# HpWang-whu/YOHO

Hardware: AMD Instinct MI355X
Metric: keypoints/sec (5000 kp x60 rot desc+YOHO-O) (higher is better)
Workload: dtype fp16x2 split (2^-22-accurate products, fp32 accumulate); 1 GPU

## Files before the change

### yoho_amd/csrc/gemmf.h

```cpp
#pragma once
#include <hip/hip_runtime.h>
#include <type_traits>
#include "common.h"

namespace yoho {

typedef float floatx16 __attribute__((ext_vector_type(16)));
typedef float floatx4 __attribute__((ext_vector_type(4)));
typedef unsigned uintx4 __attribute__((ext_vector_type(4)));
typedef _Float16 halfx8 __attribute__((ext_vector_type(8)));
typedef const __attribute__((address_space(1))) void* gptr_t;
typedef __attribute__((address_space(3))) void* lptr_t;

constexpr int FG_STAGE = 32768;
constexpr int FG_LDS = 4 * FG_STAGE;

static const int FG_ORD_D[NIR_ORD] = {5, 4, 3, 3, 1};
static const int FG_ORD_R[NIR_ORD] = {4, 3, 1, 2, 0};
static const int FG_IR_BASE[5] = {0, 1, 10, 19, 35};
static const int FG_IR_D[5] = {1, 3, 3, 4, 5};

struct FGemmArgs {
    const char* A;
    const char* B;
// ... 43 lines not shown
    int start = 0;
    for (int u = 0; u < NIR_ORD; ++u) {
        const int ru = (xcd + a.rot[u]) & 7;
        const int cnt = a.NT[u] > ru ? ((a.NT[u] - 1 - ru) / 8 + 1) * a.MT[u] : 0;
        if (slot < start + cnt) { t = u; local = slot - start; r = ru; return true; }
        start += cnt;
    }
    return false;
}

inline int fgemm_grid(const FGemmArgs& a, int per_tile) {
    int tot = 0;
    for (int x = 0; x < 8; ++x) {
        int n = 0;
        for (int t = 0; t < NIR_ORD; ++t) {
            const int r = (x + a.rot[t]) & 7;
            if (a.NT[t] > r) n += ((a.NT[t] - 1 - r) / 8 + 1) * a.MT[t] * per_tile;
        }
        tot = n > tot ? n : tot;
    }
    return 8 * tot;
}

enum { F2_NOSTORE = 0x100, F2_MIX = 0x200, F2_ST_SC1 = 0x400, F2_ST_NT = 0x800, F2_SPARSE4 = 0x1000, F2_SPARSE16 = 0x2000, F2_K32 = 0x4000 };

__device__ __forceinline__ size_t slab_off(int tile32, int q, int cout8, int o, int half, int kp32) {
    return (((((size_t)tile32 * G + q) * cout8 + (o >> 3)) * 2 + half) * TILE + kp32) * 4;
}

template <int MI, int NJ>
__device__ __forceinline__ void residual_start(floatx16 (&acc)[MI][NJ], int row0, int kp0, int jidx, int d, int qbase, const float* res, float descale,
                                               int cout, int nT32, int lane) {
    const float inv = 1.f / descale;
    const int half = lane >> 5, kp32 = lane & 31, cout8 = cout >> 3;
#pragma unroll
    for (int bi = 0; bi < NJ; ++bi) {
        const int tile32 = (kp0 >> 5) + bi;
#pragma unroll
        for (int ai = 0; ai < MI; ++ai) {
            const int rowb = row0 + ai * 32;
            const int iidx = rowb / cout, o0 = rowb - iidx * cout;
            const bool ok = tile32 < nT32 && iidx < d;
            const int q = qbase + iidx * d + jidx;
#pragma unroll
            for (int q4 = 0; q4 < 4; ++q4) {
                const size_t off = slab_off(tile32, q, cout8, o0 + q4 * 8 + half * 4, half, kp32);
                const floatx4 v = *reinterpret_cast<const floatx4*>(res + (ok ? off : 0)) * (ok ? inv : 0.f);
                acc[ai][bi][4 * q4 + 0] = v.x; acc[ai][bi][4 * q4 + 1] = v.y;
                acc[ai][bi][4 * q4 + 2] = v.z; acc[ai][bi][4 * q4 + 3] = v.w;
            }
        }
    }
}

template <int MI, int NJ>
__device__ __forceinline__ void coef_epilogue(const floatx16 (&acc)[MI][NJ], int row0, int kp0, int jidx, int d, int qbase, float* out, const float* bias,
                                              float descale, int cout, int nT32, int* rflag, int lane, int flags) {
    const int half = lane >> 5, kp32 = lane & 31, cout8 = cout >> 3;
    unsigned top = 0u;
#ifdef YOHO_EXPERIMENTS
    if ((flags & F2_SPARSE4) && (blockIdx.x >> 3) % 4 != 0) flags |= F2_NOSTORE;
    if ((flags & F2_SPARSE16) && (blockIdx.x >> 3) % 16 != 0) flags |= F2_NOSTORE;
    const __amdgpu_buffer_rsrc_t orsrc = __builtin_amdgcn_make_buffer_rsrc(out, 0, 0x7FFFFFFF, 0x00020000);
#endif
#pragma unroll
    for (int bi = 0; bi < NJ; ++bi) {
        const int tile32 = (kp0 >> 5) + bi;
        if (tile32 >= nT32) continue;
#pragma unroll
        for (int ai = 0; ai < MI; ++ai) {
            const int rowb = row0 + ai * 32;
            const int iidx = rowb / cout, o0 = rowb - iidx * cout;
            if (iidx >= d) continue;
            const int q = qbase + iidx * d + jidx;
#pragma unroll
            for (int q4 = 0; q4 < 4; ++q4) {
                const int o = o0 + q4 * 8 + half * 4;
                floatx4 val;
                val.x = acc[ai][bi][4 * q4 + 0]; val.y = acc[ai][bi][4 * q4 + 1];
                val.z = acc[ai][bi][4 * q4 + 2]; val.w = acc[ai][bi][4 * q4 + 3];
                val *= descale;
                if (d == 1) val += *reinterpret_cast<const floatx4*>(bias + o) * 7.745966692414834f;
                const size_t off = slab_off(tile32, q, cout8, o, half, kp32);
#ifdef YOHO_EXPERIMENTS
                if (flags & F2_ST_SC1) __builtin_amdgcn_raw_buffer_store_b128(__builtin_bit_cast(uintx4, val), orsrc, (int)(off * 4), 0, 16);
                else if (flags & F2_ST_NT) __builtin_amdgcn_raw_buffer_store_b128(__builtin_bit_cast(uintx4, val), orsrc, (int)(off * 4), 0, 2);
                else if (!(flags & F2_NOSTORE))
#endif
                *reinterpret_cast<floatx4*>(out + off) = val;
                top = max(max(top, __float_as_uint(val.x) & 0x7FFFFFFFu), __float_as_uint(val.y) & 0x7FFFFFFFu);
                top = max(max(top, __float_as_uint(val.z) & 0x7FFFFFFFu), __float_as_uint(val.w) & 0x7FFFFFFFu);
            }
        }
    }
    note_range_bits(rflag, top, FP16_MAX / HF_ASCALE);
}

__device__ __forceinline__ floatx4 mfma_h16(uintx4 a, uintx4 b, floatx4 c) {
    union { uintx4 u; halfx8 h; } ca, cb;
    ca.u = a; cb.u = b;
    return __builtin_amdgcn_mfma_f32_16x16x32_f16(ca.h, cb.h, c, 0, 0, 0);
}

inline bool fgemm_layer_k32(const FGemmArgs& a) { return a.cin >= 256 && a.cin % 64 == 0 && a.cout >= 256; }

template <int NJ, typename Extra>
__device__ __forceinline__ void row_products32(floatx4 (&accrow)[NJ], const uintx4& al, const uintx4& ah, const uintx4 (&bh)[NJ], const uintx4 (&bl)[NJ],
                                               Extra&& extra) {
    sfor<0, 3 * NJ>([&](auto mc) {
        constexpr int m = decltype(mc)::value, j = m % NJ, p = m / NJ;
        accrow[j] = mfma_h16(p == 0 ? al : ah, p == 1 ? bl[j] : bh[j], accrow[j]);
        __builtin_amdgcn_sched_barrier(0);
        extra(mc);
        __builtin_amdgcn_sched_barrier(0);
    });
}

template <int LOB, int MI, int NJ>
// ... 21 lines not shown
#pragma unroll
    for (int i = 0; i < MI; ++i)
#pragma unroll
        for (int j = 0; j < NJ; ++j) acc[i][j] = floatx4{0.f, 0.f, 0.f, 0.f};
}

template <bool TO_SLAB>
__device__ __forceinline__ void swap_rows16(floatx4& x, floatx4& y) {
    typedef unsigned uintx2 __attribute__((ext_vector_type(2)));
#pragma unroll
    for (int e = 0; e < 4; ++e) {
        uintx2 r = {__float_as_uint(x[e]), __float_as_uint(y[e])};
        if constexpr (TO_SLAB) {
            r = __builtin_amdgcn_permlane16_swap(r.x, r.y, false, false);
            r = __builtin_amdgcn_permlane32_swap(r.x, r.y, false, false);
        } else {
            r = __builtin_amdgcn_permlane32_swap(r.x, r.y, false, false);
            r = __builtin_amdgcn_permlane16_swap(r.x, r.y, false, false);
        }
        x[e] = __uint_as_float(r.x); y[e] = __uint_as_float(r.y);
    }
}

template <int MI, int NJ>
__device__ __forceinline__ void residual_start(floatx4 (&acc)[MI][NJ], int row0, int kp0, int jidx, int d, int qbase, const float* res, float descale,
                                               int cout, int nT32, int lane) {
    static_assert(NJ % 2 == 0, "pairs of 16-column tiles");
    const float inv = 1.f / descale;
    const int half = lane >> 5, kp32 = lane & 31, cout8 = cout >> 3;
#pragma unroll
    for (int bi = 0; bi < NJ; bi += 2) {
        const int tile32 = (kp0 >> 5) + (bi >> 1);
#pragma unroll
        for (int ai = 0; ai < MI; ++ai) {
            const int rowb = row0 + ai * 16;
            const int iidx = rowb / cout, o0 = rowb - iidx * cout;
            const bool ok = tile32 < nT32 && iidx < d;
            const int q = qbase + iidx * d + jidx;
            const size_t off0 = slab_off(tile32, q, cout8, o0 + half * 4, half, kp32), off1 = slab_off(tile32, q, cout8, o0 + 8 + half * 4, half, kp32);
            acc[ai][bi] = *reinterpret_cast<const floatx4*>(res + (ok ? off0 : 0)) * (ok ? inv : 0.f);
            acc[ai][bi + 1] = *reinterpret_cast<const floatx4*>(res + (ok ? off1 : 0)) * (ok ? inv : 0.f);
            swap_rows16<false>(acc[ai][bi], acc[ai][bi + 1]);
        }
    }
}

template <int MI, int NJ>
__device__ __forceinline__ void coef_epilogue(const floatx4 (&acc)[MI][NJ], int row0, int kp0, int jidx, int d, int qbase, float* out, const float* bias,
                                              float descale, int cout, int nT32, int* rflag, int lane, int flags) {
    static_assert(NJ % 2 == 0, "pairs of 16-column tiles");
    const int half = lane >> 5, kp32 = lane & 31, cout8 = cout >> 3;
    unsigned top = 0u;
#pragma unroll
    for (int bi = 0; bi < NJ; bi += 2) {
        const int tile32 = (kp0 >> 5) + (bi >> 1);
        if (tile32 >= nT32) continue;
#pragma unroll
        for (int ai = 0; ai < MI; ++ai) {
            const int rowb = row0 + ai * 16;
            const int iidx = rowb / cout, o0 = rowb - iidx * cout;
            if (iidx >= d) continue;
            const int q = qbase + iidx * d + jidx;
            floatx4 v[2] = {acc[ai][bi], acc[ai][bi + 1]};
            swap_rows16<true>(v[0], v[1]);
#pragma unroll
            for (int h8 = 0; h8 < 2; ++h8) {
                const int o = o0 + h8 * 8 + half * 4;
                floatx4 val = v[h8] * descale;
                if (d == 1) val += *reinterpret_cast<const floatx4*>(bias + o) * 7.745966692414834f;
#ifdef YOHO_EXPERIMENTS
                if (!(flags & F2_NOSTORE))
#endif
                *reinterpret_cast<floatx4*>(out + slab_off(tile32, q, cout8, o, half, kp32)) = val;
                top = max(max(top, __float_as_uint(val.x) & 0x7FFFFFFFu), __float_as_uint(val.y) & 0x7FFFFFFFu);
                top = max(max(top, __float_as_uint(val.z) & 0x7FFFFFFFu), __float_as_uint(val.w) & 0x7FFFFFFFu);
            }
        }
    }
    note_range_bits(rflag, top, FP16_MAX / HF_ASCALE);
}

void fgemm_fill_args(FGemmArgs& a, const Layer& L, const char* Bplanes, int kppad, int nT32, const float* res, float* out, int* rflag);
int launch_fgemm2(const FGemmArgs& a, int flags, hipStream_t s);
int launch_fgemm3(const FGemmArgs& a, int flags, hipStream_t s);
int fgemm2_init();

}
```

### yoho_amd/csrc/gemmf.hip

```cpp
#include <hip/hip_runtime.h>
#include <hip/hip_fp16.h>
#include <type_traits>
#include <vector>
#include <cmath>
#include <cstring>
#include <cstdlib>

#include "common.h"
#include "gemmf.h"

namespace yoho {

struct Frags {
    uintx4 ah[4], al[4], bh[4], bl[4];
};

template <int SUB, int R>
__device__ __forceinline__ void read_frag(const char* pa, const char* pb, Frags& f) {
    constexpr int t = R & 3;
    if constexpr (R < 4) f.al[t] = *reinterpret_cast<const uintx4*>(pa + (2 + SUB) * 8192 + t * 512);
    else if constexpr (R < 8) f.bh[t] = *reinterpret_cast<const uintx4*>(pb + (0 + SUB) * 8192 + t * 512);
    else if constexpr (R < 12) f.ah[t] = *reinterpret_cast<const uintx4*>(pa + (0 + SUB) * 8192 + t * 512);
    else f.bl[t] = *reinterpret_cast<const uintx4*>(pb + (2 + SUB) * 8192 + t * 512);
}
// ... 54 lines not shown
    const int d = a.dim[t];
    const int MT = a.MT[t], KS = d * a.cin / 32;
    const int cg = local / MT, mtile = local - cg * MT;
    const int ntile = r + 8 * cg;
    const char* Ag = a.A + a.a_off[t] + (size_t)mtile * KS * FG_STAGE;
    const char* Bg = a.B + a.b_off[t] + (size_t)ntile * KS * FG_STAGE;
    const int wm = w >> 1, wn = w & 1;
    const int lane16 = lane * 16;
    const int row0 = mtile * 256 + wm * 128;
    const int col0 = ntile * 256 + wn * 128;

    floatx16 acc[4][4];
    zero_acc(acc);

    const int lane_a = (lane >> 5) * 4096 + (wm * 128 + (lane & 31)) * 16;
    const int lane_b = FG_STAGE + (lane >> 5) * 4096 + (wn * 128 + (lane & 31)) * 16;

    stage_tile(Ag, smem, w, lane);
    stage_tile(Bg, smem + FG_STAGE, w, lane);
    if (KS > 1) {
        stage_tile(Ag + FG_STAGE, smem + 2 * FG_STAGE, w, lane);
        stage_tile(Bg + FG_STAGE, smem + 3 * FG_STAGE, w, lane);
    }
    if ((flags & EPI_RES) && row0 < d * a.cout) residual_start(acc, row0, col0 % a.kppad, col0 / a.kppad, d, a.qbase[t], a.res, a.descale, a.cout, a.nT32, lane);
    asm volatile("s_waitcnt vmcnt(0)" ::: "memory");
    __syncthreads();

    if (row0 >= d * a.cout) {
        for (int s = 0; s < KS; ++s) {
            asm volatile("s_waitcnt vmcnt(0)" ::: "memory");
            __syncthreads();
            const int s2 = s + 2 < KS ? s + 2 : KS - 1;
            char* cur = smem + (s & 1) * (2 * FG_STAGE);
            stage_tile(Ag + (size_t)s2 * FG_STAGE, cur, w, lane);
            stage_tile(Bg + (size_t)s2 * FG_STAGE, cur + FG_STAGE, w, lane);
        }
        asm volatile("s_waitcnt vmcnt(0)" ::: "memory");
        return;
    }
    Frags P, Q;
    read_frags<0>(smem + lane_a, smem + lane_b, P);
    for (int s = 0; s < KS; ++s) {
        char* cur = smem + (s & 1) * (2 * FG_STAGE);
        char* nxt = smem + ((s + 1) & 1) * (2 * FG_STAGE);
        substep<1, false>(P, acc, cur + lane_a, cur + lane_b, Q, nullptr, nullptr, nullptr, w, lane16);
        asm volatile("s_waitcnt vmcnt(0) lgkmcnt(0)" ::: "memory");
        __syncthreads();
        __builtin_amdgcn_sched_barrier(0);
        const int s2 = s + 2 < KS ? s + 2 : KS - 1;
        substep<0, true>(Q, acc, nxt + lane_a, nxt + lane_b, P, uniform_ptr(Ag + (size_t)s2 * FG_STAGE), uniform_ptr(Bg + (size_t)s2 * FG_STAGE),
                              cur, w, lane16);
    }
    asm volatile("s_waitcnt vmcnt(0)" ::: "memory");

    coef_epilogue(acc, row0, col0 % a.kppad, col0 / a.kppad, d, a.qbase[t], a.out, a.bias, a.descale, a.cout, a.nT32, a.rflag, lane, flags);
}

__global__ __launch_bounds__(256, 1) void fgemmk_kernel(FGemmArgs a, int flags) {
    extern __shared__ __attribute__((aligned(16))) char smem[];
    const int tid = threadIdx.x, lane = tid & 63;
    const int w = __builtin_amdgcn_readfirstlane(tid >> 6);
    int t = 0, local = 0, r = 0;
    if (!fg3_map(a, blockIdx.x & 7, blockIdx.x >> 3, t, local, r)) return;
    const int d = a.dim[t];
    const int MT = a.MT[t], KS = d * a.cin / 32;
    const int cg = local / MT, mtile = local - cg * MT;
    const int ntile = r + 8 * cg;
    const char* Ag = a.A + a.a_off[t] + (size_t)mtile * KS * FG_STAGE;
    const char* Bg = a.B + a.b_off[t] + (size_t)ntile * KS * FG_STAGE;
    const int wm = w >> 1, wn = w & 1;
    const int row0 = mtile * 256 + wm * 128, col0 = ntile * 256 + wn * 128;
    const bool rows_live = row0 < d * a.cout;
    const int lane_a = (lane >> 4) * 4096 + (wm * 128 + (lane & 15)) * 16;
    const int lane_b = FG_STAGE + (lane >> 4) * 4096 + (wn * 128 + (lane & 15)) * 16;

    floatx4 acc[8][8];
    zero_acc(acc);
    stage_tile(Ag, smem, w, lane);
    stage_tile(Bg, smem + FG_STAGE, w, lane);
    if (KS > 1) {
        stage_tile(Ag + FG_STAGE, smem + 2 * FG_STAGE, w, lane);
        stage_tile(Bg + FG_STAGE, smem + 3 * FG_STAGE, w, lane);
    }
    if ((flags & EPI_RES) && rows_live) residual_start(acc, row0, col0 % a.kppad, col0 / a.kppad, d, a.qbase[t], a.res, a.descale, a.cout, a.nT32, lane);
    asm volatile("s_waitcnt vmcnt(0)" ::: "memory");
    __syncthreads();
    for (int s = 0; s < KS; ++s) {
        char* cur = smem + (s & 1) * (2 * FG_STAGE);
        if (rows_live) stage32_plain<FG_STAGE / 2>(acc, cur + lane_a, cur + lane_b);
        asm volatile("s_waitcnt vmcnt(0) lgkmcnt(0)" ::: "memory");
        __syncthreads();
        __builtin_amdgcn_sched_barrier(0);
        if (s + 2 < KS) {
            stage_tile(uniform_ptr(Ag + (size_t)(s + 2) * FG_STAGE), cur, w, lane);
            stage_tile(uniform_ptr(Bg + (size_t)(s + 2) * FG_STAGE), cur + FG_STAGE, w, lane);
        }
    }
    if (rows_live) coef_epilogue(acc, row0, col0 % a.kppad, col0 / a.kppad, d, a.qbase[t], a.out, a.bias, a.descale, a.cout, a.nT32, a.rflag, lane, flags);
}

int fgemm_init() {
    HIPCHK(hipFuncSetAttribute(reinterpret_cast<const void*>(&fgemm_kernel), hipFuncAttributeMaxDynamicSharedMemorySize, FG_LDS));
    HIPCHK(hipFuncSetAttribute(reinterpret_cast<const void*>(&fgemmk_kernel), hipFuncAttributeMaxDynamicSharedMemorySize, FG_LDS));
    if (int rc = cgemm_init()) return rc;
    return fgemm2_init();
}

static long long pack_off(int t, int rows, int kdim) {
    long long off = 0;
    for (int u = 0; u < t; ++u) off += (long long)((FG_ORD_D[u] * rows + 255) / 256) * (FG_ORD_D[u] * kdim / 32) * FG_STAGE;
    return off;
}

size_t fgemm_planes_bytes(int kppad, int cin) { return (size_t)pack_off(NIR_ORD, kppad, cin); }

void fgemm_qinfo(int* qi ) {
    for (int t = 0; t < NIR_ORD; ++t) {
        const int r = FG_ORD_R[t], d = FG_IR_D[r];
        for (int m = 0; m < d; ++m)
            for (int j = 0; j < d; ++j) {
                int* p = qi + (FG_IR_BASE[r] + m * d + j) * 4;
// ... 121 lines not shown
    a.A = reinterpret_cast<const char*>(L.wpg); a.B = Bplanes; a.bias = L.bias; a.res = res; a.out = out;
    a.cin = L.cin; a.cout = L.cout; a.kppad = kppad; a.nT32 = nT32; a.descale = L.wpg_descale;
    static const int ROT[NIR_ORD] = {0, 0, 4, 4, 2};
    for (int t = 0; t < NIR_ORD; ++t) {
        a.a_off[t] = pack_off(t, L.cout, L.cin);
        a.b_off[t] = pack_off(t, kppad, L.cin);
        a.MT[t] = (FG_ORD_D[t] * L.cout + 255) / 256;
        a.NT[t] = FG_ORD_D[t] * kppad / 256;
        a.rot[t] = ROT[t];
        a.dim[t] = FG_ORD_D[t];
        a.qbase[t] = FG_IR_BASE[FG_ORD_R[t]];
    }
}

int launch_fgemm(const Layer& L, const char* Bplanes, int kppad, int nT32, const float* res, float* out, int flags, hipStream_t s, int* rflag,
                 FGemmBlocking blocking, const unsigned* amax) {
    FGemmArgs a;
    fgemm_fill_args(a, L, Bplanes, kppad, nT32, res, out, rflag);
    static const int dbg_gemm1 = [] { const char* e = experiment_env("YOHO_PARTI_DEBUG"); return (e && std::strstr(e, "gemm1")) ? 1 : 0; }();
    if (dbg_gemm1) blocking = FG_TILE256_W4;
    if (blocking == FG_TILE256_W8 && amax && L.wpg8) { a.amax = amax; a.A = reinterpret_cast<const char*>(L.wpg8); }
    const char* dbg = experiment_env("YOHO_FGEMM_DEBUG");
    if (fgemm_layer_k32(a) && !a.amax && !(dbg && std::strstr(dbg, "k16"))) flags |= F2_K32;
    if (blocking == FG_TILE256_W8) return launch_fgemm3(a, flags, s);
    if (blocking != FG_TILE256_W4) return launch_fgemm2(a, flags, s);
    if (flags & F2_K32) hipLaunchKernelGGL(fgemmk_kernel, dim3(fgemm_grid(a, 1)), dim3(256), FG_LDS, s, a, flags);
    else hipLaunchKernelGGL(fgemm_kernel, dim3(fgemm_grid(a, 1)), dim3(256), FG_LDS, s, a, flags);
    HIPCHK(hipGetLastError());
    return 0;
}

}
```

### yoho_amd/csrc/gemmf2.hip

```cpp
#include <hip/hip_runtime.h>
#include <cstdlib>
#include <cstring>
#include "common.h"
#include "gemmf.h"

namespace yoho {

constexpr int F2_BUF = 24576;
constexpr int F2_LDS = 3 * F2_BUF;
constexpr int F3_BUF = 32768;
constexpr int F3_LDS = 3 * F3_BUF;

struct Frags2 {
    uintx4 ah[4], al[4], bh[2], bl[2];
};

template <int LO, int R>
__device__ __forceinline__ void read_frag2(const char* pa, const char* pb, Frags2& f) {
    if constexpr (R < 4) f.al[R] = *reinterpret_cast<const uintx4*>(pa + 8192 + R * 512);
    else if constexpr (R < 6) f.bh[R - 4] = *reinterpret_cast<const uintx4*>(pb + (R - 4) * 512);
    else if constexpr (R < 10) f.ah[R - 6] = *reinterpret_cast<const uintx4*>(pa + (R - 6) * 512);
    else f.bl[R - 10] = *reinterpret_cast<const uintx4*>(pb + LO + (R - 10) * 512);
}
template <int LO>
// ... 140 lines not shown
    const int tid = threadIdx.x, lane = tid & 63;
    const int w = __builtin_amdgcn_readfirstlane(tid >> 6);
    int t = 0, local = 0, r = 0;
    if (!fg2_map(a, blockIdx.x & 7, blockIdx.x >> 3, (flags & F2_MIX) == 0, t, local, r)) return;
    const int d = a.dim[t];
    const int MT = a.MT[t], KS = d * a.cin / 32, KT = 2 * KS;
    const int nh = local & 1, pair = local >> 1;
    const int cg = pair / MT, mtile = pair - cg * MT;
    const int ntile = r + 8 * cg;
    const char* Ag = a.A + a.a_off[t] + (size_t)mtile * KS * FG_STAGE;
    const char* Bg = a.B + a.b_off[t] + (size_t)ntile * KS * FG_STAGE + nh * 2048;
    const int wm = w >> 1, wn = w & 1;
    const Dma2 dm(w, lane);
    const int lane_a = (lane >> 5) * 4096 + (wm * 128 + (lane & 31)) * 16;
    const int lane_b = 16384 + (lane >> 5) * 2048 + (wn * 64 + (lane & 31)) * 16;

    floatx16 acc[4][2];
    zero_acc(acc);
    auto dma = [&](int st, int buf) { dma_step(dm, Ag + step_off(st), Bg + step_off(st), smem + buf); };
    ring_prologue<F2_BUF>(KT, dma);
    const int row0 = mtile * 256 + wm * 128, colbase = ntile * 256 + nh * 128 + wn * 64;
    const bool rows_live = row0 < d * a.cout;
    const int jidx = colbase / a.kppad, kp0 = colbase - jidx * a.kppad, qbase = a.qbase[t];
    if ((flags & EPI_RES) && rows_live) residual_start(acc, row0, kp0, jidx, d, qbase, a.res, a.descale, a.cout, a.nT32, lane);
    asm volatile("s_waitcnt vmcnt(0)" ::: "memory");
    __builtin_amdgcn_s_barrier();
    if (!rows_live) return ring_pipelined_idle<F2_BUF>(KT, dma);

    Frags2 P;
    read_frags2<Dma2::LO>(smem + lane_a, smem + lane_b, P);
    ring_pipelined<F2_BUF, 6>(smem, Ag, Bg, KT, lane_a, lane_b, P,
        [&](auto dmac, const Frags2& f, Frags2& nf, const char* ra, const char* rb, const char* srcA, const char* srcB, char* buf) {
            step2<decltype(dmac)::value>(dm, f, acc, ra, rb, nf, srcA, srcB, buf);
        });
    coef_epilogue(acc, row0, kp0, jidx, d, qbase, a.out, a.bias, a.descale, a.cout, a.nT32, a.rflag, lane, flags);
}

struct Wave3 {
    int wm, wn, nh, lane_a, lane_b;
    Dma3 dm;
    __device__ __forceinline__ Wave3(int w8, int lane) : wm((w8 & 3) >> 1), wn(w8 & 1), nh(w8 >> 2), dm(w8, lane) {
        lane_a = (lane >> 5) * 4096 + (wm * 128 + (lane & 31)) * 16;
        lane_b = 16384 + (lane >> 5) * 4096 + (nh * 128 + wn * 64 + (lane & 31)) * 16;
    }
};

__global__ __launch_bounds__(512, 2) void fgemm3_kernel(FGemmArgs a, int flags) {
    extern __shared__ __attribute__((aligned(16))) char smem[];
    const int tid = threadIdx.x, lane = tid & 63;
    const Wave3 wv(__builtin_amdgcn_readfirstlane(tid >> 6), lane);
    int t = 0, local = 0, r = 0;
    if (!fg3_map(a, blockIdx.x & 7, blockIdx.x >> 3, t, local, r)) return;
    const int d = a.dim[t];
    const int MT = a.MT[t], KS = d * a.cin / 32, KT = 2 * KS;
    const int cg = local / MT, mtile = local - cg * MT;
    const int ntile = r + 8 * cg;
    const char* Ag = a.A + a.a_off[t] + (size_t)mtile * KS * FG_STAGE;
    const char* Bg = a.B + a.b_off[t] + (size_t)ntile * KS * FG_STAGE;

    floatx16 acc[4][2];
    zero_acc(acc);
    auto dma = [&](int st, int buf) { dma_step(wv.dm, Ag + step_off(st), Bg + step_off(st), smem + buf); };
    ring_prologue<F3_BUF>(KT, dma);
    const int row0 = mtile * 256 + wv.wm * 128, colbase = ntile * 256 + wv.nh * 128 + wv.wn * 64;
    const bool rows_live = row0 < d * a.cout;
    const int jidx = colbase / a.kppad, kp0 = colbase - jidx * a.kppad, qbase = a.qbase[t];
    if ((flags & EPI_RES) && rows_live) residual_start(acc, row0, kp0, jidx, d, qbase, a.res, a.descale, a.cout, a.nT32, lane);
    asm volatile("s_waitcnt vmcnt(0)" ::: "memory");
    __builtin_amdgcn_s_barrier();
    if (!rows_live) return ring_pipelined_idle<F3_BUF>(KT, dma);

    Frags2 P;
    read_frags2<Dma3::LO>(smem + wv.lane_a, smem + wv.lane_b, P);
    ring_pipelined<F3_BUF, 4>(smem, Ag, Bg, KT, wv.lane_a, wv.lane_b, P,
        [&](auto dmac, const Frags2& f, Frags2& nf, const char* ra, const char* rb, const char* srcA, const char* srcB, char* buf) {
            step2<decltype(dmac)::value>(wv.dm, f, acc, ra, rb, nf, srcA, srcB, buf);
        });
    coef_epilogue(acc, row0, kp0, jidx, d, qbase, a.out, a.bias, a.descale, a.cout, a.nT32, a.rflag, lane, flags);
}

constexpr int F3K_BUF = 2 * FG_STAGE;
constexpr int F3K_LDS = 2 * F3K_BUF;

struct Dma3k {
    static constexpr int NP = 8;
    int la, ldst;
    __device__ __forceinline__ Dma3k(int w8, int lane) : la(w8 * 1024 + lane * 16), ldst(w8 * 1024) {}
    template <int U>
    __device__ __forceinline__ void piece(const char* srcA, const char* srcB, char* buf) const {
        constexpr int q = (U & 3) * 8192;
        if constexpr (U < 4) __builtin_amdgcn_global_load_lds((gptr_t)(srcA + q + la), (lptr_t)(buf + q + ldst), 16, 0, 0);
        else __builtin_amdgcn_global_load_lds((gptr_t)(srcB + q + la), (lptr_t)(buf + FG_STAGE + q + ldst), 16, 0, 0);
    }
};
struct FragsA32 { uintx4 al, ah; };
struct FragsB32 { uintx4 bh[4], bl[4]; };

template <int R>
__device__ __forceinline__ void read_open32(const char* pa, const char* pb, FragsA32& a0, FragsB32& b) {
    if constexpr (R == 0) a0.al = *reinterpret_cast<const uintx4*>(pa + 16384);
    else if constexpr (R < 5) b.bh[R - 1] = *reinterpret_cast<const uintx4*>(pb + (R - 1) * 256);
// ... 34 lines not shown
    const int d = a.dim[t];
    const int MT = a.MT[t], KS = d * a.cin / 32;
    const int cg = local / MT, mtile = local - cg * MT;
    const int ntile = r + 8 * cg;
    const char* Ag = a.A + a.a_off[t] + (size_t)mtile * KS * FG_STAGE;
    const char* Bg = a.B + a.b_off[t] + (size_t)ntile * KS * FG_STAGE;
    const int wm = (w8 & 3) >> 1, wn = w8 & 1, nh = w8 >> 2;
    const Dma3k dm(w8, lane);
    const int lane_a = (lane >> 4) * 4096 + (wm * 128 + (lane & 15)) * 16;
    const int lane_b = FG_STAGE + (lane >> 4) * 4096 + (nh * 128 + wn * 64 + (lane & 15)) * 16;

    floatx4 acc[8][4];
    zero_acc(acc);
    auto dma = [&](int st, int buf) {
        const char* sa = uniform_ptr(Ag + (size_t)st * FG_STAGE);
        const char* sb = uniform_ptr(Bg + (size_t)st * FG_STAGE);
        sfor<0, Dma3k::NP>([&](auto uc) { dm.template piece<decltype(uc)::value>(sa, sb, smem + buf); });
    };
    dma(0, 0);
    if (KS > 1) dma(1, F3K_BUF);
    const int row0 = mtile * 256 + wm * 128, colbase = ntile * 256 + nh * 128 + wn * 64;
    const bool rows_live = row0 < d * a.cout;
    const int jidx = colbase / a.kppad, kp0 = colbase - jidx * a.kppad, qbase = a.qbase[t];
    if ((flags & EPI_RES) && rows_live) residual_start(acc, row0, kp0, jidx, d, qbase, a.res, a.descale, a.cout, a.nT32, lane);
    asm volatile("s_waitcnt vmcnt(0)" ::: "memory");
    __builtin_amdgcn_s_barrier();
    if (!rows_live) {
        for (int s = 0; s < KS; ++s) {
            asm volatile("s_waitcnt vmcnt(0)" ::: "memory");
            __builtin_amdgcn_s_barrier();
            if (s + 2 < KS) dma(s + 2, (s & 1) * F3K_BUF);
        }
        asm volatile("s_waitcnt vmcnt(0)" ::: "memory");
        return;
    }

    FragsA32 fa[2];
    FragsB32 P, Q;
    sfor<0, 10>([&](auto rc) { read_open32<decltype(rc)::value>(smem + lane_a, smem + lane_b, fa[0], P); });
    int s = 0, cur = 0;
    auto run = [&](auto dmac, const FragsB32& b, FragsB32& nb) {
        const int nxt = cur ^ F3K_BUF;
        if constexpr (decltype(dmac)::value)
            step32<true>(dm, acc, fa, b, nb, smem + cur + lane_a, smem + nxt + lane_a, smem + nxt + lane_b, uniform_ptr(Ag + (size_t)(s + 2) * FG_STAGE),
                         uniform_ptr(Bg + (size_t)(s + 2) * FG_STAGE), smem + cur);
        else
            step32<false>(dm, acc, fa, b, nb, smem + cur + lane_a, smem + nxt + lane_a, smem + nxt + lane_b, nullptr, nullptr, nullptr);
        cur = nxt; ++s;
    };
    constexpr std::true_type dmay;
    constexpr std::false_type dman;
    while (s + 2 < KS) {
        run(dmay, P, Q);
        run(dmay, Q, P);
    }
    run(dman, P, Q);
    run(dman, Q, P);
    coef_epilogue(acc, row0, kp0, jidx, d, qbase, a.out, a.bias, a.descale, a.cout, a.nT32, a.rflag, lane, flags);
}

constexpr int F2K_BUF = FG_STAGE + FG_STAGE / 2;
constexpr int F2K_LDS = 2 * F2K_BUF;

__global__ __launch_bounds__(256, 1) void fgemm2k_kernel(FGemmArgs a, int flags) {
    extern __shared__ __attribute__((aligned(16))) char smem[];
    const int tid = threadIdx.x, lane = tid & 63;
    const int w = __builtin_amdgcn_readfirstlane(tid >> 6);
    int t = 0, local = 0, r = 0;
    if (!fg2_map(a, blockIdx.x & 7, blockIdx.x >> 3, (flags & F2_MIX) == 0, t, local, r)) return;
    const int d = a.dim[t];
    const int MT = a.MT[t], KS = d * a.cin / 32;
    const int nh = local & 1, pair = local >> 1;
    const int cg = pair / MT, mtile = pair - cg * MT;
    const int ntile = r + 8 * cg;
    const char* Ag = a.A + a.a_off[t] + (size_t)mtile * KS * FG_STAGE;
    const char* Bg = a.B + a.b_off[t] + (size_t)ntile * KS * FG_STAGE + nh * 2048;
    const int wm = w >> 1, wn = w & 1;
    const int lane_a = (lane >> 4) * 4096 + (wm * 128 + (lane & 15)) * 16;
    const int lane_b = FG_STAGE + (lane >> 4) * 2048 + (wn * 64 + (lane & 15)) * 16;

    floatx4 acc[8][4];
    zero_acc(acc);
    auto dma = [&](int st, int buf) {
        const char* sa = uniform_ptr(Ag + (size_t)st * FG_STAGE) + lane * 16;
        const char* sb = uniform_ptr(Bg + (size_t)st * FG_STAGE) + lane * 16;
#pragma unroll
        for (int k = 0; k < 8; ++k) __builtin_amdgcn_global_load_lds((gptr_t)(sa + (k * 4 + w) * 1024), (lptr_t)(smem + buf + (k * 4 + w) * 1024), 16, 0, 0);
#pragma unroll
        for (int k = 0; k < 4; ++k) {
            const int pb = w * 4 + k, u = pb >> 1, part = pb & 1;
            __builtin_amdgcn_global_load_lds((gptr_t)(sb + u * 4096 + part * 1024), (lptr_t)(smem + buf + FG_STAGE + u * 2048 + part * 1024), 16, 0, 0);
        }
    };
    dma(0, 0);
    if (KS > 1) dma(1, F2K_BUF);
    const int row0 = mtile * 256 + wm * 128, colbase = ntile * 256 + nh * 128 + wn * 64;
    const bool rows_live = row0 < d * a.cout;
    const int jidx = colbase / a.kppad, kp0 = colbase - jidx * a.kppad, qbase = a.qbase[t];
    if ((flags & EPI_RES) && rows_live) residual_start(acc, row0, kp0, jidx, d, qbase, a.res, a.descale, a.cout, a.nT32, lane);
    asm volatile("s_waitcnt vmcnt(0)" ::: "memory");
    __builtin_amdgcn_s_barrier();
    for (int s = 0; s < KS; ++s) {
        const int cur = (s & 1) * F2K_BUF;
        if (rows_live) stage32_plain<FG_STAGE / 4>(acc, smem + cur + lane_a, smem + cur + lane_b);
        asm volatile("s_waitcnt vmcnt(0) lgkmcnt(0)" ::: "memory");
        __builtin_amdgcn_s_barrier();
        __builtin_amdgcn_sched_barrier(0);
        if (s + 2 < KS) dma(s + 2, cur);
    }
    if (rows_live) coef_epilogue(acc, row0, kp0, jidx, d, qbase, a.out, a.bias, a.descale, a.cout, a.nT32, a.rflag, lane, flags);
}

typedef int intx8 __attribute__((ext_vector_type(8)));
typedef short shortx2 __attribute__((ext_vector_type(2)));
typedef _Float16 halfx2 __attribute__((ext_vector_type(2)));
struct Frags8 {
    intx8 a[4], b[2];
};
struct C8Scales {
    float ah = 4.f, al = 4.f / 2048.f, bh = 1.f, bl = 1.f;
    int mfma_b = 127;
    C8Scales() = default;
    __device__ __forceinline__ explicit C8Scales(const unsigned* amax) {
        const unsigned amax_bits = __builtin_amdgcn_readfirstlane(*amax);
        int kexp = (int)(amax_bits >> 23) - 127 - 7;
        kexp = kexp < -60 ? -60 : (kexp > 9 ? 9 : kexp);
        bh = __uint_as_float((unsigned)(kexp + 127) << 23); bl = __uint_as_float((unsigned)(kexp - 11 + 127) << 23);
        mfma_b = 127 + kexp;
    }
};
struct Int2 { int x, y; };
__device__ __forceinline__ Int2 frag_to_fp8(uintx4 f, float scale) {
    union { unsigned u; halfx2 h; } p0, p1, p2, p3;
// ... 95 lines not shown
}

__global__ __launch_bounds__(512, 2) void fgemm3c_kernel(FGemmArgs a, int flags) {
    extern __shared__ __attribute__((aligned(16))) char smem[];
    const int tid = threadIdx.x, lane = tid & 63;
    const Wave3 wv(__builtin_amdgcn_readfirstlane(tid >> 6), lane);
    int t = 0, local = 0, r = 0;
    if (!fg3_map(a, blockIdx.x & 7, blockIdx.x >> 3, t, local, r)) return;
    const int d = a.dim[t];
    const int MT = a.MT[t], KS = d * a.cin / 32, KT = 2 * KS;
    const int cg = local / MT, mtile = local - cg * MT;
    const int ntile = r + 8 * cg;
    const char* Ag = a.A + a.a_off[t] + (size_t)mtile * KS * FG_STAGE;
    const char* Bg = a.B + a.b_off[t] + (size_t)ntile * KS * FG_STAGE;

    floatx16 acc[4][2];
    zero_acc(acc);
    const C8Scales sc(a.amax);
    dma_step(wv.dm, Ag, Bg, smem);
    dma_step(wv.dm, Ag + step_off(1), Bg + step_off(1), smem + F3_BUF);
    const int row0 = mtile * 256 + wv.wm * 128, colbase = ntile * 256 + wv.nh * 128 + wv.wn * 64;
    const bool rows_live = row0 < d * a.cout;
    const int jidx = colbase / a.kppad, kp0 = colbase - jidx * a.kppad, qbase = a.qbase[t];
    if ((flags & EPI_RES) && rows_live) residual_start(acc, row0, kp0, jidx, d, qbase, a.res, a.descale, a.cout, a.nT32, lane);
    asm volatile("s_waitcnt vmcnt(0)" ::: "memory");
    __builtin_amdgcn_s_barrier();

    ring_plain<true>(acc, smem, wv, Ag, [&](int s) { return Bg + step_off(s); }, KT, rows_live, sc);
    if (rows_live) coef_epilogue(acc, row0, kp0, jidx, d, qbase, a.out, a.bias, a.descale, a.cout, a.nT32, a.rflag, lane, flags);
}

struct CGemmArgs {
    const char* A;
    const char* B;
    const float* bias;
    const float* bn_s;
    const float* bn_t;
    char* out;
    int NTm, MT, KSt, ntap, nj, nslot, c8out, nT32, nTiles16;
    float descale;
    int* rflag;
    const unsigned* amax;
    unsigned char slot[13 * 13];
    unsigned char outg[16];
};

__device__ __forceinline__ void cg_split_pair(float x0, float x1, unsigned& hi, unsigned& lo) {
    typedef float f2 __attribute__((ext_vector_type(2)));
    f2 x;
    x.x = x0; x.y = x1;
    const halfx2 h = __builtin_convertvector(x, halfx2);
    const f2 r = x - __builtin_convertvector(h, f2);
// ... 154 lines not shown
    const int d = a.dim[t];
    const int KS = d * a.cin / 32, KT = 2 * KS;
    const int ntile = r + 8 * local;
    const char* Ag = a.A + a.a_off[t];
    const char* Bg = a.B + a.b_off[t] + (size_t)ntile * KS * FG_STAGE;
    const Dma3 dm(w8, lane);
    const int lane_a = (lane >> 5) * 4096 + (lane & 31) * 16;
    const int lane_b = 16384 + (lane >> 5) * 4096 + (w8 * 32 + (lane & 31)) * 16;

    floatx16 acc[5][1];
    zero_acc(acc);
    ring_prologue<F3_BUF>(KT, [&](int st, int buf) { dma_step(dm, uniform_ptr(Ag + step_off(st)), uniform_ptr(Bg + step_off(st)), smem + buf); });
    asm volatile("s_waitcnt vmcnt(0)" ::: "memory");
    __builtin_amdgcn_s_barrier();

    switch (d) {
        case 1: fgemm3s_kloop<1>(acc, smem, Ag, Bg, KT, dm, lane_a, lane_b); break;
        case 3: fgemm3s_kloop<3>(acc, smem, Ag, Bg, KT, dm, lane_a, lane_b); break;
        case 4: fgemm3s_kloop<4>(acc, smem, Ag, Bg, KT, dm, lane_a, lane_b); break;
        default: fgemm3s_kloop<5>(acc, smem, Ag, Bg, KT, dm, lane_a, lane_b); break;
    }
    const int colbase = ntile * 256 + w8 * 32;
    const int jidx = colbase / a.kppad, kp0 = colbase - jidx * a.kppad;
    coef_epilogue(acc, 0, kp0, jidx, d, a.qbase[t], a.out, a.bias, a.descale, 32, a.nT32, a.rflag, lane, flags & F2_NOSTORE);
}

int fgemm3_init() {
    HIPCHK(hipFuncSetAttribute(reinterpret_cast<const void*>(&fgemm3_kernel), hipFuncAttributeMaxDynamicSharedMemorySize, F3_LDS));
    HIPCHK(hipFuncSetAttribute(reinterpret_cast<const void*>(&fgemm3s_kernel), hipFuncAttributeMaxDynamicSharedMemorySize, F3_LDS));
    HIPCHK(hipFuncSetAttribute(reinterpret_cast<const void*>(&fgemm3c_kernel), hipFuncAttributeMaxDynamicSharedMemorySize, F3_LDS));
    HIPCHK(hipFuncSetAttribute(reinterpret_cast<const void*>(&fgemm3k_kernel), hipFuncAttributeMaxDynamicSharedMemorySize, F3K_LDS));
    return 0;
}

int launch_fgemm3(const FGemmArgs& a, int flags, hipStream_t s) {
    if (const char* dbg = experiment_env("YOHO_FGEMM_DEBUG")) {
        if (std::strstr(dbg, "nostore")) flags |= F2_NOSTORE;
        if (std::strstr(dbg, "sc1")) flags |= F2_ST_SC1;
        if (std::strstr(dbg, "stnt")) flags |= F2_ST_NT;
    }
    const int tot = fgemm_grid(a, 1);
    static const bool small_ok = [] { const char* e = experiment_env("YOHO_FGEMM_DEBUG"); return !(e && std::strstr(e, "nosmall")); }();
    if (small_ok && a.cout == 32 && !(flags & EPI_RES)) hipLaunchKernelGGL(fgemm3s_kernel, dim3(tot), dim3(512), F3_LDS, s, a, flags);
    else if (a.amax) hipLaunchKernelGGL(fgemm3c_kernel, dim3(tot), dim3(512), F3_LDS, s, a, flags);
    else if (flags & F2_K32) hipLaunchKernelGGL(fgemm3k_kernel, dim3(tot), dim3(512), F3K_LDS, s, a, flags);
    else hipLaunchKernelGGL(fgemm3_kernel, dim3(tot), dim3(512), F3_LDS, s, a, flags);
    HIPCHK(hipGetLastError());
// ... 26 lines not shown
```

Before: 1.889 million keypoints/s.

## Fuse residual add into GEMM epilogue with prefetched ring instead of accumulator preload

```diff
diff --git a/yoho_amd/csrc/gemmf.h b/yoho_amd/csrc/gemmf.h
--- a/yoho_amd/csrc/gemmf.h
+++ b/yoho_amd/csrc/gemmf.h
@@ -89,12 +89,23 @@
     return 8 * tot;
 }
 
-enum { F2_NOSTORE = 0x100, F2_MIX = 0x200, F2_ST_SC1 = 0x400, F2_ST_NT = 0x800, F2_SPARSE4 = 0x1000, F2_SPARSE16 = 0x2000, F2_K32 = 0x4000 };
+enum { F2_NOSTORE = 0x100, F2_MIX = 0x200, F2_ST_SC1 = 0x400, F2_ST_NT = 0x800, F2_SPARSE4 = 0x1000, F2_SPARSE16 = 0x2000, F2_K32 = 0x4000,
+       F2_RESSTART = 0x8000 };
 
 __device__ __forceinline__ size_t slab_off(int tile32, int q, int cout8, int o, int half, int kp32) {
     return (((((size_t)tile32 * G + q) * cout8 + (o >> 3)) * 2 + half) * TILE + kp32) * 4;
 }
 
+constexpr int RES_AHEAD = 8;
+__device__ __forceinline__ bool epi_has_res(int flags) { return (flags & EPI_RES) && !(flags & F2_RESSTART); }
+template <bool RES>
+__device__ __forceinline__ floatx4 epi_value(floatx4 acc, float descale, floatx4 r) {
+    if constexpr (!RES) return acc * descale;
+    else return floatx4{__builtin_fmaf(acc.x, descale, r.x), __builtin_fmaf(acc.y, descale, r.y), __builtin_fmaf(acc.z, descale, r.z),
+                   __builtin_fmaf(acc.w, descale, r.w)};
+}
+
+#ifdef YOHO_EXPERIMENTS
 template <int MI, int NJ>
 __device__ __forceinline__ void residual_start(floatx16 (&acc)[MI][NJ], int row0, int kp0, int jidx, int d, int qbase, const float* res, float descale,
                                                int cout, int nT32, int lane) {
@@ -119,10 +130,12 @@
         }
     }
 }
-
-template <int MI, int NJ>
-__device__ __forceinline__ void coef_epilogue(const floatx16 (&acc)[MI][NJ], int row0, int kp0, int jidx, int d, int qbase, float* out, const float* bias,
-                                              float descale, int cout, int nT32, int* rflag, int lane, int flags) {
+#endif
+
+template <bool FAST, bool RES, int MI, int NJ>
+__device__ __forceinline__ void coef_epilogue_body(const floatx16 (&acc)[MI][NJ], int row0, int kp0, int jidx, int d, int qbase, float* out, const float* res,
+                                                   const float* bias, float descale, int cout, int nT32, int* rflag, int lane, int flags) {
+    constexpr int N = 4 * MI * NJ;
     const int half = lane >> 5, kp32 = lane & 31, cout8 = cout >> 3;
     unsigned top = 0u;
 #ifdef YOHO_EXPERIMENTS
@@ -130,37 +143,73 @@
     if ((flags & F2_SPARSE16) && (blockIdx.x >> 3) % 16 != 0) flags |= F2_NOSTORE;
     const __amdgpu_buffer_rsrc_t orsrc = __builtin_amdgcn_make_buffer_rsrc(out, 0, 0x7FFFFFFF, 0x00020000);
 #endif
-#pragma unroll
-    for (int bi = 0; bi < NJ; ++bi) {
+    int iidx[MI], o0[MI];
+#pragma unroll
+    for (int ai = 0; ai < MI; ++ai) {
+        const int rowb = row0 + ai * 32;
+        iidx[ai] = rowb / cout; o0[ai] = rowb - iidx[ai] * cout;
+    }
+    auto where = [&](auto kc, int& o, size_t& off) {
+        constexpr int k = decltype(kc)::value, bi = k / (4 * MI), ai = (k / 4) % MI, q4 = k & 3;
         const int tile32 = (kp0 >> 5) + bi;
-        if (tile32 >= nT32) continue;
-#pragma unroll
-        for (int ai = 0; ai < MI; ++ai) {
-            const int rowb = row0 + ai * 32;
-            const int iidx = rowb / cout, o0 = rowb - iidx * cout;
-            if (iidx >= d) continue;
-            const int q = qbase + iidx * d + jidx;
-#pragma unroll
-            for (int q4 = 0; q4 < 4; ++q4) {
-                const int o = o0 + q4 * 8 + half * 4;
-                floatx4 val;
-                val.x = acc[ai][bi][4 * q4 + 0]; val.y = acc[ai][bi][4 * q4 + 1];
-                val.z = acc[ai][bi][4 * q4 + 2]; val.w = acc[ai][bi][4 * q4 + 3];
-                val *= descale;
+        o = o0[ai] + q4 * 8 + half * 4;
+        off = slab_off(tile32, qbase + iidx[ai] * d + jidx, cout8, o, half, kp32);
+        return FAST || (tile32 < nT32 && iidx[ai] < d);
+    };
+    floatx4 ring[RES_AHEAD];
+    auto fetch = [&](auto kc) {
+        constexpr int k = decltype(kc)::value;
+        if constexpr (RES && k < N) {
+            int o; size_t off;
+            if (where(kc, o, off)) ring[k % RES_AHEAD] = *reinterpret_cast<const floatx4*>(res + off);
+        }
+    };
+    sfor<0, RES_AHEAD>(fetch);
+    sfor<0, N>([&](auto kc) {
+        constexpr int k = decltype(kc)::value, bi = k / (4 * MI), ai = (k / 4) % MI, q4 = k & 3;
+        int o; size_t off;
+        if (where(kc, o, off)) {
+            floatx4 val;
+            val.x = acc[ai][bi][4 * q4 + 0]; val.y = acc[ai][bi][4 * q4 + 1];
+            val.z = acc[ai][bi][4 * q4 + 2]; val.w = acc[ai][bi][4 * q4 + 3];
+            val = epi_value<RES>(val, descale, ring[k % RES_AHEAD]);
+            if constexpr (!FAST)
                 if (d == 1) val += *reinterpret_cast<const floatx4*>(bias + o) * 7.745966692414834f;
-                const size_t off = slab_off(tile32, q, cout8, o, half, kp32);
-#ifdef YOHO_EXPERIMENTS
-                if (flags & F2_ST_SC1) __builtin_amdgcn_raw_buffer_store_b128(__builtin_bit_cast(uintx4, val), orsrc, (int)(off * 4), 0, 16);
-                else if (flags & F2_ST_NT) __builtin_amdgcn_raw_buffer_store_b128(__builtin_bit_cast(uintx4, val), orsrc, (int)(off * 4), 0, 2);
-                else if (!(flags & F2_NOSTORE))
-#endif
-                *reinterpret_cast<floatx4*>(out + off) = val;
-                top = max(max(top, __float_as_uint(val.x) & 0x7FFFFFFFu), __float_as_uint(val.y) & 0x7FFFFFFFu);
-                top = max(max(top, __float_as_uint(val.z) & 0x7FFFFFFFu), __float_as_uint(val.w) & 0x7FFFFFFFu);
-            }
-        }
-    }
+#ifdef YOHO_EXPERIMENTS
+            if (flags & F2_ST_SC1) __builtin_amdgcn_raw_buffer_store_b128(__builtin_bit_cast(uintx4, val), orsrc, (int)(off * 4), 0, 16);
+            else if (flags & F2_ST_NT) __builtin_amdgcn_raw_buffer_store_b128(__builtin_bit_cast(uintx4, val), orsrc, (int)(off * 4), 0, 2);
+            else if (!(flags & F2_NOSTORE))
+#endif
+            *reinterpret_cast<floatx4*>(out + off) = val;
+            top = max(max(top, __float_as_uint(val.x) & 0x7FFFFFFFu), __float_as_uint(val.y) & 0x7FFFFFFFu);
+            top = max(max(top, __float_as_uint(val.z) & 0x7FFFFFFFu), __float_as_uint(val.w) & 0x7FFFFFFFu);
+        }
+        fetch(std::integral_constant<int, k + RES_AHEAD>{});
+        if constexpr (FAST) __builtin_amdgcn_sched_barrier(0);
+    });
     note_range_bits(rflag, top, FP16_MAX / HF_ASCALE);
+}
+
+template <bool FAST, bool RES, int MI, int NJ>
+__device__ __forceinline__ void coef_epilogue_body(const floatx4 (&acc)[MI][NJ], int row0, int kp0, int jidx, int d, int qbase, float* out, const float* res,
+                                                   const float* bias, float descale, int cout, int nT32, int* rflag, int lane, int flags);
+
+template <int ROWS, int TILES32, int MI, int NJ, typename Acc>
+__device__ __forceinline__ void coef_epilogue_dispatch(const Acc (&acc)[MI][NJ], int row0, int kp0, int jidx, int d, int qbase, float* out, const float* res,
+                                                       const float* bias, float descale, int cout, int nT32, int* rflag, int lane, int flags) {
+    const bool fast = d != 1 && (kp0 >> 5) + TILES32 <= nT32 && (row0 + (MI - 1) * ROWS) / cout < d;
+    auto run = [&](auto fastc, auto resc) {
+        coef_epilogue_body<decltype(fastc)::value, decltype(resc)::value>(acc, row0, kp0, jidx, d, qbase, out, res, bias, descale, cout, nT32, rflag, lane, flags);
+    };
+    constexpr std::true_type yes;
+    constexpr std::false_type no;
+    if (epi_has_res(flags)) { if (fast) run(yes, yes); else run(no, yes); }
+    else { if (fast) run(yes, no); else run(no, no); }
+}
+template <int MI, int NJ>
+__device__ __forceinline__ void coef_epilogue(const floatx16 (&acc)[MI][NJ], int row0, int kp0, int jidx, int d, int qbase, float* out, const float* res,
+                                              const float* bias, float descale, int cout, int nT32, int* rflag, int lane, int flags) {
+    coef_epilogue_dispatch<32, NJ>(acc, row0, kp0, jidx, d, qbase, out, res, bias, descale, cout, nT32, rflag, lane, flags);
 }
 
 __device__ __forceinline__ floatx4 mfma_h16(uintx4 a, uintx4 b, floatx4 c) {
@@ -228,6 +277,7 @@
     }
 }
 
+#ifdef YOHO_EXPERIMENTS
 template <int MI, int NJ>
 __device__ __forceinline__ void residual_start(floatx4 (&acc)[MI][NJ], int row0, int kp0, int jidx, int d, int qbase, const float* res, float descale,
                                                int cout, int nT32, int lane) {
@@ -250,40 +300,79 @@
         }
     }
 }
-
-template <int MI, int NJ>
-__device__ __forceinline__ void coef_epilogue(const floatx4 (&acc)[MI][NJ], int row0, int kp0, int jidx, int d, int qbase, float* out, const float* bias,
-                                              float descale, int cout, int nT32, int* rflag, int lane, int flags) {
-    static_assert(NJ % 2 == 0, "pairs of 16-column tiles");
+#endif
+
+template <typename Acc>
+__device__ __forceinline__ void resstart_experiment(Acc& acc, int flags, bool rows_live, int row0, int kp0, int jidx, int d, int qbase, const float* res,
+                                                    float descale, int cout, int nT32, int lane) {
+#ifdef YOHO_EXPERIMENTS
+    if ((flags & EPI_RES) && (flags & F2_RESSTART) && rows_live) residual_start(acc, row0, kp0, jidx, d, qbase, res, descale, cout, nT32, lane);
+#endif
+}
+
+template <bool FAST, bool RES, int MI, int NJ>
+__device__ __forceinline__ void coef_epilogue_body(const floatx4 (&acc)[MI][NJ], int row0, int kp0, int jidx, int d, int qbase, float* out, const float* res,
+                                                   const float* bias, float descale, int cout, int nT32, int* rflag, int lane, int flags) {
+    static_assert(NJ % 2 == 0 && RES_AHEAD % 2 == 0, "pairs of 16-column tiles");
+    constexpr int N = MI * NJ / 2, AHEAD = RES_AHEAD / 2;
     const int half = lane >> 5, kp32 = lane & 31, cout8 = cout >> 3;
     unsigned top = 0u;
-#pragma unroll
-    for (int bi = 0; bi < NJ; bi += 2) {
-        const int tile32 = (kp0 >> 5) + (bi >> 1);
-        if (tile32 >= nT32) continue;
-#pragma unroll
-        for (int ai = 0; ai < MI; ++ai) {
-            const int rowb = row0 + ai * 16;
-            const int iidx = rowb / cout, o0 = rowb - iidx * cout;
-            if (iidx >= d) continue;
-            const int q = qbase + iidx * d + jidx;
+    int iidx[MI], o0[MI];
+#pragma unroll
+    for (int ai = 0; ai < MI; ++ai) {
+        const int rowb = row0 + ai * 16;
+        iidx[ai] = rowb / cout; o0[ai] = rowb - iidx[ai] * cout;
+    }
+    auto where = [&](auto kc, int (&o)[2], size_t (&off)[2]) {
+        constexpr int k = decltype(kc)::value, ai = k % MI;
+        const int tile32 = (kp0 >> 5) + k / MI;
+#pragma unroll
+        for (int h8 = 0; h8 < 2; ++h8) {
+            o[h8] = o0[ai] + h8 * 8 + half * 4;
+            off[h8] = slab_off(tile32, qbase + iidx[ai] * d + jidx, cout8, o[h8], half, kp32);
+        }
+        return FAST || (tile32 < nT32 && iidx[ai] < d);
+    };
+    floatx4 ring[AHEAD][2];
+    auto fetch = [&](auto kc) {
+        constexpr int k = decltype(kc)::value;
+        if constexpr (RES && k < N) {
+            int o[2]; size_t off[2];
+            if (where(kc, o, off)) {
+                ring[k % AHEAD][0] = *reinterpret_cast<const floatx4*>(res + off[0]);
+                ring[k % AHEAD][1] = *reinterpret_cast<const floatx4*>(res + off[1]);
+            }
+        }
+    };
+    sfor<0, AHEAD>(fetch);
+    sfor<0, N>([&](auto kc) {
+        constexpr int k = decltype(kc)::value, bi = (k / MI) * 2, ai = k % MI;
+        int o[2]; size_t off[2];
+        if (where(kc, o, off)) {
             floatx4 v[2] = {acc[ai][bi], acc[ai][bi + 1]};
             swap_rows16<true>(v[0], v[1]);
 #pragma unroll
             for (int h8 = 0; h8 < 2; ++h8) {
-                const int o = o0 + h8 * 8 + half * 4;
-                floatx4 val = v[h8] * descale;
-                if (d == 1) val += *reinterpret_cast<const floatx4*>(bias + o) * 7.745966692414834f;
+                floatx4 val = epi_value<RES>(v[h8], descale, ring[k % AHEAD][h8]);
+                if constexpr (!FAST)
+                    if (d == 1) val += *reinterpret_cast<const floatx4*>(bias + o[h8]) * 7.745966692414834f;
 #ifdef YOHO_EXPERIMENTS
                 if (!(flags & F2_NOSTORE))
 #endif
-                *reinterpret_cast<floatx4*>(out + slab_off(tile32, q, cout8, o, half, kp32)) = val;
+                *reinterpret_cast<floatx4*>(out + off[h8]) = val;
                 top = max(max(top, __float_as_uint(val.x) & 0x7FFFFFFFu), __float_as_uint(val.y) & 0x7FFFFFFFu);
                 top = max(max(top, __float_as_uint(val.z) & 0x7FFFFFFFu), __float_as_uint(val.w) & 0x7FFFFFFFu);
             }
         }
-    }
+        fetch(std::integral_constant<int, k + AHEAD>{});
+        if constexpr (FAST) __builtin_amdgcn_sched_barrier(0);
+    });
     note_range_bits(rflag, top, FP16_MAX / HF_ASCALE);
+}
+template <int MI, int NJ>
+__device__ __forceinline__ void coef_epilogue(const floatx4 (&acc)[MI][NJ], int row0, int kp0, int jidx, int d, int qbase, float* out, const float* res,
+                                              const float* bias, float descale, int cout, int nT32, int* rflag, int lane, int flags) {
+    coef_epilogue_dispatch<16, NJ / 2>(acc, row0, kp0, jidx, d, qbase, out, res, bias, descale, cout, nT32, rflag, lane, flags);
 }
 
 void fgemm_fill_args(FGemmArgs& a, const Layer& L, const char* Bplanes, int kppad, int nT32, const float* res, float* out, int* rflag);
diff --git a/yoho_amd/csrc/gemmf.hip b/yoho_amd/csrc/gemmf.hip
--- a/yoho_amd/csrc/gemmf.hip
+++ b/yoho_amd/csrc/gemmf.hip
@@ -100,7 +100,7 @@
         stage_tile(Ag + FG_STAGE, smem + 2 * FG_STAGE, w, lane);
         stage_tile(Bg + FG_STAGE, smem + 3 * FG_STAGE, w, lane);
     }
-    if ((flags & EPI_RES) && row0 < d * a.cout) residual_start(acc, row0, col0 % a.kppad, col0 / a.kppad, d, a.qbase[t], a.res, a.descale, a.cout, a.nT32, lane);
+    resstart_experiment(acc, flags, row0 < d * a.cout, row0, col0 % a.kppad, col0 / a.kppad, d, a.qbase[t], a.res, a.descale, a.cout, a.nT32, lane);
     asm volatile("s_waitcnt vmcnt(0)" ::: "memory");
     __syncthreads();
 
@@ -131,7 +131,7 @@
     }
     asm volatile("s_waitcnt vmcnt(0)" ::: "memory");
 
-    coef_epilogue(acc, row0, col0 % a.kppad, col0 / a.kppad, d, a.qbase[t], a.out, a.bias, a.descale, a.cout, a.nT32, a.rflag, lane, flags);
+    coef_epilogue(acc, row0, col0 % a.kppad, col0 / a.kppad, d, a.qbase[t], a.out, a.res, a.bias, a.descale, a.cout, a.nT32, a.rflag, lane, flags);
 }
 
 __global__ __launch_bounds__(256, 1) void fgemmk_kernel(FGemmArgs a, int flags) {
@@ -160,7 +160,7 @@
         stage_tile(Ag + FG_STAGE, smem + 2 * FG_STAGE, w, lane);
         stage_tile(Bg + FG_STAGE, smem + 3 * FG_STAGE, w, lane);
     }
-    if ((flags & EPI_RES) && rows_live) residual_start(acc, row0, col0 % a.kppad, col0 / a.kppad, d, a.qbase[t], a.res, a.descale, a.cout, a.nT32, lane);
+    resstart_experiment(acc, flags, rows_live, row0, col0 % a.kppad, col0 / a.kppad, d, a.qbase[t], a.res, a.descale, a.cout, a.nT32, lane);
     asm volatile("s_waitcnt vmcnt(0)" ::: "memory");
     __syncthreads();
     for (int s = 0; s < KS; ++s) {
@@ -174,7 +174,7 @@
             stage_tile(uniform_ptr(Bg + (size_t)(s + 2) * FG_STAGE), cur + FG_STAGE, w, lane);
         }
     }
-    if (rows_live) coef_epilogue(acc, row0, col0 % a.kppad, col0 / a.kppad, d, a.qbase[t], a.out, a.bias, a.descale, a.cout, a.nT32, a.rflag, lane, flags);
+    if (rows_live) coef_epilogue(acc, row0, col0 % a.kppad, col0 / a.kppad, d, a.qbase[t], a.out, a.res, a.bias, a.descale, a.cout, a.nT32, a.rflag, lane, flags);
 }
 
 int fgemm_init() {
@@ -342,6 +342,7 @@
     if (blocking == FG_TILE256_W8 && amax && L.wpg8) { a.amax = amax; a.A = reinterpret_cast<const char*>(L.wpg8); }
     const char* dbg = experiment_env("YOHO_FGEMM_DEBUG");
     if (fgemm_layer_k32(a) && !a.amax && !(dbg && std::strstr(dbg, "k16"))) flags |= F2_K32;
+    if (dbg && std::strstr(dbg, "resstart")) flags |= F2_RESSTART;
     if (blocking == FG_TILE256_W8) return launch_fgemm3(a, flags, s);
     if (blocking != FG_TILE256_W4) return launch_fgemm2(a, flags, s);
     if (flags & F2_K32) hipLaunchKernelGGL(fgemmk_kernel, dim3(fgemm_grid(a, 1)), dim3(256), FG_LDS, s, a, flags);
diff --git a/yoho_amd/csrc/gemmf2.hip b/yoho_amd/csrc/gemmf2.hip
--- a/yoho_amd/csrc/gemmf2.hip
+++ b/yoho_amd/csrc/gemmf2.hip
@@ -186,7 +186,7 @@
     const int row0 = mtile * 256 + wm * 128, colbase = ntile * 256 + nh * 128 + wn * 64;
     const bool rows_live = row0 < d * a.cout;
     const int jidx = colbase / a.kppad, kp0 = colbase - jidx * a.kppad, qbase = a.qbase[t];
-    if ((flags & EPI_RES) && rows_live) residual_start(acc, row0, kp0, jidx, d, qbase, a.res, a.descale, a.cout, a.nT32, lane);
+    resstart_experiment(acc, flags, rows_live, row0, kp0, jidx, d, qbase, a.res, a.descale, a.cout, a.nT32, lane);
     asm volatile("s_waitcnt vmcnt(0)" ::: "memory");
     __builtin_amdgcn_s_barrier();
     if (!rows_live) return ring_pipelined_idle<F2_BUF>(KT, dma);
@@ -197,7 +197,7 @@
         [&](auto dmac, const Frags2& f, Frags2& nf, const char* ra, const char* rb, const char* srcA, const char* srcB, char* buf) {
             step2<decltype(dmac)::value>(dm, f, acc, ra, rb, nf, srcA, srcB, buf);
         });
-    coef_epilogue(acc, row0, kp0, jidx, d, qbase, a.out, a.bias, a.descale, a.cout, a.nT32, a.rflag, lane, flags);
+    coef_epilogue(acc, row0, kp0, jidx, d, qbase, a.out, a.res, a.bias, a.descale, a.cout, a.nT32, a.rflag, lane, flags);
 }
 
 struct Wave3 {
@@ -229,7 +229,7 @@
     const int row0 = mtile * 256 + wv.wm * 128, colbase = ntile * 256 + wv.nh * 128 + wv.wn * 64;
     const bool rows_live = row0 < d * a.cout;
     const int jidx = colbase / a.kppad, kp0 = colbase - jidx * a.kppad, qbase = a.qbase[t];
-    if ((flags & EPI_RES) && rows_live) residual_start(acc, row0, kp0, jidx, d, qbase, a.res, a.descale, a.cout, a.nT32, lane);
+    resstart_experiment(acc, flags, rows_live, row0, kp0, jidx, d, qbase, a.res, a.descale, a.cout, a.nT32, lane);
     asm volatile("s_waitcnt vmcnt(0)" ::: "memory");
     __builtin_amdgcn_s_barrier();
     if (!rows_live) return ring_pipelined_idle<F3_BUF>(KT, dma);
@@ -240,7 +240,7 @@
         [&](auto dmac, const Frags2& f, Frags2& nf, const char* ra, const char* rb, const char* srcA, const char* srcB, char* buf) {
             step2<decltype(dmac)::value>(wv.dm, f, acc, ra, rb, nf, srcA, srcB, buf);
         });
-    coef_epilogue(acc, row0, kp0, jidx, d, qbase, a.out, a.bias, a.descale, a.cout, a.nT32, a.rflag, lane, flags);
+    coef_epilogue(acc, row0, kp0, jidx, d, qbase, a.out, a.res, a.bias, a.descale, a.cout, a.nT32, a.rflag, lane, flags);
 }
 
 constexpr int F3K_BUF = 2 * FG_STAGE;
@@ -321,7 +321,7 @@
     const int row0 = mtile * 256 + wm * 128, colbase = ntile * 256 + nh * 128 + wn * 64;
     const bool rows_live = row0 < d * a.cout;
     const int jidx = colbase / a.kppad, kp0 = colbase - jidx * a.kppad, qbase = a.qbase[t];
-    if ((flags & EPI_RES) && rows_live) residual_start(acc, row0, kp0, jidx, d, qbase, a.res, a.descale, a.cout, a.nT32, lane);
+    resstart_experiment(acc, flags, rows_live, row0, kp0, jidx, d, qbase, a.res, a.descale, a.cout, a.nT32, lane);
     asm volatile("s_waitcnt vmcnt(0)" ::: "memory");
     __builtin_amdgcn_s_barrier();
     if (!rows_live) {
@@ -355,7 +355,7 @@
     }
     run(dman, P, Q);
     run(dman, Q, P);
-    coef_epilogue(acc, row0, kp0, jidx, d, qbase, a.out, a.bias, a.descale, a.cout, a.nT32, a.rflag, lane, flags);
+    coef_epilogue(acc, row0, kp0, jidx, d, qbase, a.out, a.res, a.bias, a.descale, a.cout, a.nT32, a.rflag, lane, flags);
 }
 
 constexpr int F2K_BUF = FG_STAGE + FG_STAGE / 2;
@@ -396,7 +396,7 @@
     const int row0 = mtile * 256 + wm * 128, colbase = ntile * 256 + nh * 128 + wn * 64;
     const bool rows_live = row0 < d * a.cout;
     const int jidx = colbase / a.kppad, kp0 = colbase - jidx * a.kppad, qbase = a.qbase[t];
-    if ((flags & EPI_RES) && rows_live) residual_start(acc, row0, kp0, jidx, d, qbase, a.res, a.descale, a.cout, a.nT32, lane);
+    resstart_experiment(acc, flags, rows_live, row0, kp0, jidx, d, qbase, a.res, a.descale, a.cout, a.nT32, lane);
     asm volatile("s_waitcnt vmcnt(0)" ::: "memory");
     __builtin_amdgcn_s_barrier();
     for (int s = 0; s < KS; ++s) {
@@ -407,7 +407,7 @@
         __builtin_amdgcn_sched_barrier(0);
         if (s + 2 < KS) dma(s + 2, cur);
     }
-    if (rows_live) coef_epilogue(acc, row0, kp0, jidx, d, qbase, a.out, a.bias, a.descale, a.cout, a.nT32, a.rflag, lane, flags);
+    if (rows_live) coef_epilogue(acc, row0, kp0, jidx, d, qbase, a.out, a.res, a.bias, a.descale, a.cout, a.nT32, a.rflag, lane, flags);
 }
 
 typedef int intx8 __attribute__((ext_vector_type(8)));
@@ -549,12 +549,12 @@
     const int row0 = mtile * 256 + wv.wm * 128, colbase = ntile * 256 + wv.nh * 128 + wv.wn * 64;
     const bool rows_live = row0 < d * a.cout;
     const int jidx = colbase / a.kppad, kp0 = colbase - jidx * a.kppad, qbase = a.qbase[t];
-    if ((flags & EPI_RES) && rows_live) residual_start(acc, row0, kp0, jidx, d, qbase, a.res, a.descale, a.cout, a.nT32, lane);
+    resstart_experiment(acc, flags, rows_live, row0, kp0, jidx, d, qbase, a.res, a.descale, a.cout, a.nT32, lane);
     asm volatile("s_waitcnt vmcnt(0)" ::: "memory");
     __builtin_amdgcn_s_barrier();
 
     ring_plain<true>(acc, smem, wv, Ag, [&](int s) { return Bg + step_off(s); }, KT, rows_live, sc);
-    if (rows_live) coef_epilogue(acc, row0, kp0, jidx, d, qbase, a.out, a.bias, a.descale, a.cout, a.nT32, a.rflag, lane, flags);
+    if (rows_live) coef_epilogue(acc, row0, kp0, jidx, d, qbase, a.out, a.res, a.bias, a.descale, a.cout, a.nT32, a.rflag, lane, flags);
 }
 
 struct CGemmArgs {
@@ -755,7 +755,7 @@
     }
     const int colbase = ntile * 256 + w8 * 32;
     const int jidx = colbase / a.kppad, kp0 = colbase - jidx * a.kppad;
-    coef_epilogue(acc, 0, kp0, jidx, d, a.qbase[t], a.out, a.bias, a.descale, 32, a.nT32, a.rflag, lane, flags & F2_NOSTORE);
+    coef_epilogue(acc, 0, kp0, jidx, d, a.qbase[t], a.out, nullptr, a.bias, a.descale, 32, a.nT32, a.rflag, lane, flags & F2_NOSTORE);
 }
 
 int fgemm3_init() {
```

New measurement: 1.895 million keypoints/s (median of 6 runs). No clear change (+0.3%).
